# 610265158/Peppa_Pig_Face_Landmark

Measured on NVIDIA H100. Metric: faces/sec Student@256 batch=256, higher is better.
Workload: dtype f32

## Files before the change

### peppa_pig_face_landmark_b200/csrc/conv_tct.cu

```cuda
#include <cuda.h>
#include <cuda_fp16.h>
#include <math.h>
#include <string.h>

#include <algorithm>

#include "../../include/skps_b200.h"
#include "common.h"
#include "conv_tct.h"
#include "tc_ptx.h"

namespace skps {

constexpr int TCT_THREADS = 288;
constexpr int TCT_M = 128, TCT_N = 256;
constexpr int TCT_KC = 32;
constexpr int TCT_W_PLANE = TCT_M * 2 * TCT_KC;
constexpr int TCT_W_SLOT = 2 * TCT_W_PLANE;
constexpr int TCT_W_SLOTS = 3;
constexpr int TCT_MAX_X_SLOTS = 3;
constexpr int TCT_OUT_BYTES = 2 * 16384;
constexpr int TCT_SMEM_LIMIT = 227 * 1024 - 256;

template <int ACT>
__global__ void __launch_bounds__(TCT_THREADS, 1)
conv_tct_kernel(const __grid_constant__ CUtensorMap tmX_hi, const __grid_constant__ CUtensorMap tmX_lo,
                const __grid_constant__ CUtensorMap tmW_hi, const __grid_constant__ CUtensorMap tmW_lo,
                const __grid_constant__ CUtensorMap tmO_hi, const __grid_constant__ CUtensorMap tmO_lo, const TctK p) {
    extern __shared__ uint8_t smem_raw[];
    __shared__ __align__(8) uint64_t full_w[TCT_W_SLOTS], empty_w[TCT_W_SLOTS], full_x[TCT_MAX_X_SLOTS],
        empty_x[TCT_MAX_X_SLOTS];

    const int warp = threadIdx.x >> 5, lane = threadIdx.x & 31;
    const uint32_t base = (smem_u32(smem_raw) + 1023u) & ~1023u;
    const uint32_t x_base = base + (uint32_t)TCT_W_SLOTS * TCT_W_SLOT;
    const uint32_t x_slot = 2u * (uint32_t)p.x_plane;
    const uint32_t out_off = x_base + (uint32_t)p.x_slots * x_slot;
    const int tiles = p.m_tiles;
    const int kh = p.taps / p.kw;
    const int halves = (p.Cin + TCT_KC - 1) / TCT_KC;
    const int groups = p.kw * halves;

    if (warp == 8 && lane == 0) {
        asm volatile("prefetch.tensormap [%0];" ::"l"(&tmX_hi) : "memory");
        asm volatile("prefetch.tensormap [%0];" ::"l"(&tmX_lo) : "memory");
        asm volatile("prefetch.tensormap [%0];" ::"l"(&tmW_hi) : "memory");
        asm volatile("prefetch.tensormap [%0];" ::"l"(&tmW_lo) : "memory");
    }
    if (warp == 1 && lane == 0) {
        for (int s = 0; s < TCT_W_SLOTS; ++s) {
            mbar_init(smem_u32(&full_w[s]), 1);
            mbar_init(smem_u32(&empty_w[s]), 8);
        }
        for (int s = 0; s < p.x_slots; ++s) {
            mbar_init(smem_u32(&full_x[s]), 1);
            mbar_init(smem_u32(&empty_x[s]), 8);
        }
        asm volatile("fence.mbarrier_init.release.cluster;" ::: "memory");
    }
    __syncthreads();

    if (warp == 8) {
        if (lane == 0 && (int)blockIdx.x < tiles) {
            const int total = ((tiles - (int)blockIdx.x + (int)gridDim.x - 1) / (int)gridDim.x) * groups;
            int xs = 0, ws = 0;
            uint32_t xphase = 0, wphase = 0;
            auto load_halo = [&](int n) {
                const int i = n / groups, g = n - i * groups;
                const int kx = g / halves, hc = g - kx * halves;
                const int tile = (int)blockIdx.x + i * (int)gridDim.x;
                const int img_l = tile / p.tiles_per_img, t = tile - img_l * p.tiles_per_img;
                mbar_wait(smem_u32(&empty_x[xs]), xphase ^ 1u);
                const uint32_t fb = smem_u32(&full_x[xs]);
                mbar_expect_tx(fb, x_slot);
                const uint32_t sx = x_base + (uint32_t)xs * x_slot;
                const int cx = kx * p.dil - p.pad, cy = t * p.bh - p.pad;
                tma_load_4d(sx, &tmX_hi, fb, hc * TCT_KC, cx, cy, img_l + p.img0);
                tma_load_4d(sx + (uint32_t)p.x_plane, &tmX_lo, fb, hc * TCT_KC, cx, cy, img_l + p.img0);
                if (++xs == p.x_slots) { xs = 0; xphase ^= 1u; }
            };
            load_halo(0);
            for (int n = 0, g = 0; n < total; ++n) {
                const int kx = g / halves, hc = g - kx * halves;
                for (int ky = 0; ky < kh; ++ky) {
                    mbar_wait(smem_u32(&empty_w[ws]), wphase ^ 1u);
                    const uint32_t fb = smem_u32(&full_w[ws]);
                    mbar_expect_tx(fb, (uint32_t)TCT_W_SLOT);
                    const uint32_t sw = base + (uint32_t)ws * TCT_W_SLOT;
                    const int col = (ky * p.kw + kx) * p.cchunks * 64 + hc * TCT_KC;
                    tma_load_2d(sw, &tmW_hi, fb, col, 0);
                    tma_load_2d(sw + TCT_W_PLANE, &tmW_lo, fb, col, 0);
                    if (++ws == TCT_W_SLOTS) { ws = 0; wphase ^= 1u; }
                    if (ky == 0 && n + 1 < total) load_halo(n + 1);
                }
                if (++g == groups) g = 0;
            }
        }
    } else {
        const int q = warp & 3;
        const int half_id = warp >> 2;
        const bool leader = q == 0 && lane == 0;
        float bias[4];
#pragma unroll
        for (int r = 0; r < 4; ++r) {
            const int c = 64 * (r >> 1) + 16 * q + (lane >> 2) + 8 * (r & 1);
            bias[r] = c < p.Cout ? __ldg(p.bias + c) : 0.f;
        }
        const uint32_t sbuf = out_off + (uint32_t)half_id * 16384u;
        uint32_t row_addr[4];
#pragma unroll
        for (int r = 0; r < 4; ++r) {
            const int cq = 16 * (q & 1) + (lane >> 2) + 8 * (r & 1);
            row_addr[r] = sbuf + (uint32_t)(2 * (r >> 1) + (q >> 1)) * 4096u + (uint32_t)(2 * (lane & 3)) * 64u +
                          (uint32_t)((((cq >> 3) ^ (lane & 3)) & 3) << 4) + (uint32_t)(cq & 7) * 2u;
        }
        const int ks_last = (p.Cin - (halves - 1) * TCT_KC + 15) / 16;
        const uint32_t tap_step = (uint32_t)(p.dil * p.W * 2 * TCT_KC);
        int xs = 0, ws = 0;
        uint32_t xphase = 0, wphase = 0;
        for (int tile = blockIdx.x; tile < tiles; tile += gridDim.x) {
            const int img_l = tile / p.tiles_per_img, t = tile - img_l * p.tiles_per_img;
            float acc[128];
            int prev_w = -1, prev_x = -1;
            for (int g = 0, hc = 0; g < groups; ++g) {
                mbar_wait(smem_u32(&full_x[xs]), xphase);
                const uint32_t xo = x_base + (uint32_t)xs * x_slot + (uint32_t)(half_id * 128 * 2 * TCT_KC);
                const bool two = hc != halves - 1 || ks_last == 2;
                for (int ky = 0; ky < kh; ++ky) {
                    mbar_wait(smem_u32(&full_w[ws]), wphase);
                    const uint32_t sw = base + (uint32_t)ws * TCT_W_SLOT;
                    const uint64_t w_hi = make_smem_desc_sw64(sw), w_lo = make_smem_desc_sw64(sw + TCT_W_PLANE);
                    const uint32_t xk = xo + (uint32_t)ky * tap_step;
                    const uint64_t x_hi = make_smem_desc_sw64(xk), x_lo = make_smem_desc_sw64(xk + (uint32_t)p.x_plane);
                    const uint32_t accumulate = (g | ky) != 0;
                    wg_fence_acc(acc);
                    if (two) {
                        wg_fence(); wg_mma3_128x128<2, 64>(acc, w_hi, w_lo, x_hi, x_lo, accumulate); wg_commit();
                    } else {
                        wg_fence(); wg_mma3_128x128<1, 64>(acc, w_hi, w_lo, x_hi, x_lo, accumulate); wg_commit();
                    }
                    wg_fence_acc(acc);
                    wg_wait<1>();
                    wg_fence_acc(acc);
                    if (lane == 0) {
                        if (prev_w >= 0) mbar_arrive(smem_u32(&empty_w[prev_w]));
                        if (prev_x >= 0) mbar_arrive(smem_u32(&empty_x[prev_x]));
                    }
                    prev_w = ws;
                    prev_x = ky == kh - 1 ? xs : -1;
                    if (++ws == TCT_W_SLOTS) { ws = 0; wphase ^= 1u; }
                }
                if (++xs == p.x_slots) { xs = 0; xphase ^= 1u; }
                if (++hc == halves) hc = 0;
            }
            wg_wait<0>();
            wg_fence_acc(acc);
            if (lane == 0) {
                mbar_arrive(smem_u32(&empty_w[prev_w]));
                mbar_arrive(smem_u32(&empty_x[prev_x]));
            }
#pragma unroll
            for (int ci = 0; ci < 4; ++ci) {
                if (leader) asm volatile("cp.async.bulk.wait_group.read 0;" ::: "memory");
                asm volatile("bar.sync %0, 128;" ::"r"(5 + half_id) : "memory");
#pragma unroll
                for (int m = 0; m < 2; ++m)
#pragma unroll
                    for (int i = 0; i < 4; ++i)
#pragma unroll
                        for (int e = 0; e < 4; ++e) {
                            const float f = act_t<ACT>(fmaf(acc[64 * m + 16 * ci + 4 * i + e], p.out_scale, bias[2 * m + (e >> 1)]));
                            const __half h = __float2half_rn(f);
                            const __half l = __float2half_rn(f - __half2float(h));
                            const uint32_t a = row_addr[2 * m + (e >> 1)] + (uint32_t)(8 * i + (e & 1)) * 64u;
                            asm volatile("st.shared.b16 [%0], %1;" ::"r"(a), "h"(__half_as_ushort(h)) : "memory");
                            asm volatile("st.shared.b16 [%0], %1;" ::"r"(a + 2048u), "h"(__half_as_ushort(l)) : "memory");
                        }
                asm volatile("fence.proxy.async.shared::cta;" ::: "memory");
                asm volatile("bar.sync %0, 128;" ::"r"(5 + half_id) : "memory");
                if (leader) {
                    const int col0 = half_id * 128 + ci * 32;
                    const int x0 = col0 % p.W, y0 = t * p.bh + col0 / p.W;
                    for (int cq = 0; cq < 4 && cq * 32 < p.Cout; ++cq) {
                        const uint32_t sq = sbuf + (uint32_t)cq * 4096u;
                        asm volatile("cp.async.bulk.tensor.4d.global.shared::cta.bulk_group [%0, {%2, %3, %4, %5}], [%1];"
                                     ::"l"(&tmO_hi), "r"(sq), "r"(cq * 32), "r"(x0), "r"(y0), "r"(img_l + p.img0) : "memory");
                        asm volatile("cp.async.bulk.tensor.4d.global.shared::cta.bulk_group [%0, {%2, %3, %4, %5}], [%1];"
                                     ::"l"(&tmO_lo), "r"(sq + 2048u), "r"(cq * 32), "r"(x0), "r"(y0), "r"(img_l + p.img0) : "memory");
                    }
                    asm volatile("cp.async.bulk.commit_group;" ::: "memory");
                }
            }
        }
        if (leader) asm volatile("cp.async.bulk.wait_group 0;" ::: "memory");
    }
}

static int tct_x_plane(const TcSetup& s) { return (TCT_N / s.W + s.dil * (s.kh - 1)) * s.W * 2 * TCT_KC; }
static int tct_x_slots(const TcSetup& s) {
    const int room = TCT_SMEM_LIMIT - 1024 - TCT_W_SLOTS * TCT_W_SLOT - TCT_OUT_BYTES;
    return std::min(TCT_MAX_X_SLOTS, room / (2 * tct_x_plane(s)));
}

bool tct_applicable(const TcSetup& s) {
    const int stride = s.stride > 0 ? s.stride : 1;
    if (stride != 1 || s.kh != s.kw || s.kh < 3 || s.pad != s.dil * (s.kh - 1) / 2) return false;
    if (s.W < 16 || s.W > TCT_N || TCT_N % s.W || s.H % (TCT_N / s.W)) return false;
    if (s.Cin < 64 || (s.Cin % 8) || (s.in_ld % 8) || (s.in_coff % 8)) return false;
    if (s.Cout < 96 || s.Cout > TCT_M || (s.Cout % 8) || s.n_tiles != 1) return false;
    if (s.res || s.hm_val || s.out_fmt != DT_SPLIT16 || s.out_cstride != 1 || (s.out_ld % 8) || (s.out_coff % 8)) return false;
    if (s.act == ACT_SILU) return false;
    return tct_x_slots(s) >= 2;
}

int tct_prepare(TctLayer& L, const TcSetup& s) {
    EncodeTiledFn enc = tensor_map_encoder();
    SKPS_CHECK(enc, "cuTensorMapEncodeTiled entry point not available");
    SKPS_CHECK(tct_applicable(s), "conv_tct: layer not applicable");
    TctK& k = L.k;
    memset(&k, 0, sizeof(k));
    k.W = s.W; k.bh = TCT_N / s.W; k.tiles_per_img = s.H / k.bh;
    k.taps = s.kh * s.kw; k.kw = s.kw; k.dil = s.dil; k.pad = s.pad;
    k.cchunks = (s.Cin + 63) / 64; k.Cin = s.Cin; k.Cout = s.Cout; k.act = s.act; k.out_scale = s.out_scale;
    SKPS_CHECK(s.bias, "conv_tct: bias required");
    k.bias = s.bias;
    k.x_plane = tct_x_plane(s); k.x_slots = tct_x_slots(s);
    L.smem_bytes = 1024 + TCT_W_SLOTS * TCT_W_SLOT + k.x_slots * 2 * k.x_plane + TCT_OUT_BYTES;
    for (int plane = 0; plane < 2; ++plane) {
        cuuint64_t dims[4] = {(cuuint64_t)s.Cin, (cuuint64_t)s.W, (cuuint64_t)s.H, (cuuint64_t)s.max_batch};
        cuuint64_t strides[3] = {(cuuint64_t)s.in_ld * 2, (cuuint64_t)s.W * s.in_ld * 2, (cuuint64_t)s.H * s.W * s.in_ld * 2};
        cuuint32_t box[4] = {TCT_KC, (cuuint32_t)s.W, (cuuint32_t)(k.bh + s.dil * (s.kh - 1)), 1};
        cuuint32_t estr[4] = {1, 1, 1, 1};
        void* base = (void*)((__half*)s.in_base + (plane ? s.in_plane : 0) + s.in_coff);
        CUresult r = enc(plane ? &L.x_lo : &L.x_hi, CU_TENSOR_MAP_DATA_TYPE_FLOAT16, 4, base, dims, strides, box, estr,
                         CU_TENSOR_MAP_INTERLEAVE_NONE, CU_TENSOR_MAP_SWIZZLE_64B,
                         CU_TENSOR_MAP_L2_PROMOTION_L2_128B, CU_TENSOR_MAP_FLOAT_OOB_FILL_NONE);
        SKPS_CHECK(r == CUDA_SUCCESS, "cuTensorMapEncodeTiled(tct X) failed: %d", (int)r);
    }
    const int K_pad = k.taps * k.cchunks * 64;
    for (int plane = 0; plane < 2; ++plane) {
        cuuint64_t dims[2] = {(cuuint64_t)K_pad, (cuuint64_t)s.n_tile};
        cuuint64_t strides[1] = {(cuuint64_t)K_pad * 2};
        cuuint32_t box[2] = {TCT_KC, (cuuint32_t)TCT_M};
        cuuint32_t estr[2] = {1, 1};
        void* base = (void*)(plane ? s.w_lo : s.w_hi);
        CUresult r = enc(plane ? &L.w_lo : &L.w_hi, CU_TENSOR_MAP_DATA_TYPE_FLOAT16, 2, base, dims, strides, box, estr,
                         CU_TENSOR_MAP_INTERLEAVE_NONE, CU_TENSOR_MAP_SWIZZLE_64B,
                         CU_TENSOR_MAP_L2_PROMOTION_L2_256B, CU_TENSOR_MAP_FLOAT_OOB_FILL_NONE);
        SKPS_CHECK(r == CUDA_SUCCESS, "cuTensorMapEncodeTiled(tct W) failed: %d", (int)r);
    }
    for (int plane = 0; plane < 2; ++plane) {
        cuuint64_t dims[4] = {(cuuint64_t)s.Cout, (cuuint64_t)s.W, (cuuint64_t)s.H, (cuuint64_t)s.max_batch};
        cuuint64_t strides[3] = {(cuuint64_t)s.out_ld * 2, (cuuint64_t)s.W * s.out_ld * 2, (cuuint64_t)s.H * s.W * s.out_ld * 2};
        const cuuint32_t obw = (cuuint32_t)(s.W < 32 ? s.W : 32);
        cuuint32_t box[4] = {32, obw, 32 / obw, 1};
        cuuint32_t estr[4] = {1, 1, 1, 1};
        char* base = (char*)s.out + (size_t)s.out_coff * 2 + (plane ? (size_t)s.out_plane * 2 : 0);
        CUresult r = enc(plane ? &L.o_lo : &L.o_hi, CU_TENSOR_MAP_DATA_TYPE_FLOAT16, 4, base, dims, strides, box, estr,
                         CU_TENSOR_MAP_INTERLEAVE_NONE, CU_TENSOR_MAP_SWIZZLE_64B, CU_TENSOR_MAP_L2_PROMOTION_NONE,
                         CU_TENSOR_MAP_FLOAT_OOB_FILL_NONE);
        SKPS_CHECK(r == CUDA_SUCCESS, "cuTensorMapEncodeTiled(tct out) failed: %d", (int)r);
    }
    return 0;
}

template <int ACT>
static int tct_launch_t(const TctLayer& L, const TctK& k, int grid, cudaStream_t stream) {
    static int attr_bytes[MAX_DEVICES] = {};
    if (smem_limit((const void*)conv_tct_kernel<ACT>, attr_bytes, L.smem_bytes)) return 1;
    conv_tct_kernel<ACT><<<grid, TCT_THREADS, L.smem_bytes, stream>>>(L.x_hi, L.x_lo, L.w_hi, L.w_lo, L.o_hi, L.o_lo, k);
    SKPS_CUDA(cudaGetLastError());
    return 0;
}

Grid tct_grid(const TctLayer& L, int batch, int num_sms, TctK* kp) {
    TctK k = L.k;
    k.m_tiles = batch * k.tiles_per_img;
    if (kp) *kp = k;
    return persistent_grid(k.m_tiles, num_sms);
}

int tct_launch(const TctLayer& L, int batch, int num_sms, cudaStream_t stream) {
    TctK k;
    const int grid = tct_grid(L, batch, num_sms, &k).ctas;
    switch (k.act) {
        case ACT_NONE: return tct_launch_t<ACT_NONE>(L, k, grid, stream);
        case ACT_RELU: return tct_launch_t<ACT_RELU>(L, k, grid, stream);
        case ACT_HSWISH: return tct_launch_t<ACT_HSWISH>(L, k, grid, stream);
        case ACT_SIGMOID: return tct_launch_t<ACT_SIGMOID>(L, k, grid, stream);
        case ACT_HSIGMOID: return tct_launch_t<ACT_HSIGMOID>(L, k, grid, stream);
        default: break;
    }
    set_error("conv_tct: activation %d not instantiated", k.act);
    return 1;
}

}
```

Baseline: 20180.

## Multicast conv weight tiles across 2-CTA clusters and shrink output staging

Result: faster. 20510, median of 6 (+1.7%).

```diff
diff --git a/peppa_pig_face_landmark_b200/csrc/conv_tct.cu b/peppa_pig_face_landmark_b200/csrc/conv_tct.cu
--- a/peppa_pig_face_landmark_b200/csrc/conv_tct.cu
+++ b/peppa_pig_face_landmark_b200/csrc/conv_tct.cu
@@ -17,10 +17,42 @@
 constexpr int TCT_KC = 32;
 constexpr int TCT_W_PLANE = TCT_M * 2 * TCT_KC;
 constexpr int TCT_W_SLOT = 2 * TCT_W_PLANE;
-constexpr int TCT_W_SLOTS = 3;
+constexpr int TCT_W_SLOTS = 4;
 constexpr int TCT_MAX_X_SLOTS = 3;
-constexpr int TCT_OUT_BYTES = 2 * 16384;
+constexpr int TCT_OUT_BYTES = 2 * 8192;
 constexpr int TCT_SMEM_LIMIT = 227 * 1024 - 256;
+constexpr int TCT_CLUSTER = 2;
+constexpr int TCT_W_ROWS = TCT_M / TCT_CLUSTER;
+constexpr int TCT_W_BOX = TCT_W_ROWS * 2 * TCT_KC;
+
+__device__ __forceinline__ uint32_t cluster_ctarank() {
+    uint32_t r;
+    asm volatile("mov.u32 %0, %%cluster_ctarank;" : "=r"(r));
+    return r;
+}
+__device__ __forceinline__ uint32_t cluster_nctarank() {
+    uint32_t r;
+    asm volatile("mov.u32 %0, %%cluster_nctarank;" : "=r"(r));
+    return r;
+}
+__device__ __forceinline__ void cluster_sync() {
+    asm volatile("barrier.cluster.arrive.release;\n\tbarrier.cluster.wait.acquire;" ::: "memory");
+}
+__device__ __forceinline__ void mbar_arrive_remote(uint32_t bar, uint32_t rank) {
+    asm volatile(
+        "{\n\t"
+        ".reg .b32 ra;\n\t"
+        "mapa.shared::cluster.u32 ra, %0, %1;\n\t"
+        "mbarrier.arrive.shared::cluster.b64 _, [ra];\n\t"
+        "}\n" ::"r"(bar), "r"(rank) : "memory");
+}
+__device__ __forceinline__ void tma_load_2d_multicast(uint32_t dst, const CUtensorMap* map, uint32_t bar, int c0, int c1,
+                                                      uint16_t mask) {
+    asm volatile(
+        "cp.async.bulk.tensor.2d.shared::cluster.global.mbarrier::complete_tx::bytes.multicast::cluster"
+        " [%0], [%1, {%3, %4}], [%2], %5;"
+        ::"r"(dst), "l"(map), "r"(bar), "r"(c0), "r"(c1), "h"(mask) : "memory");
+}
 
 template <int ACT>
 __global__ void __launch_bounds__(TCT_THREADS, 1)
@@ -40,6 +72,10 @@
     const int kh = p.taps / p.kw;
     const int halves = (p.Cin + TCT_KC - 1) / TCT_KC;
     const int groups = p.kw * halves;
+    const uint32_t nc = cluster_nctarank(), rank = cluster_ctarank();
+    const int grid = (int)gridDim.x;
+    const int mine = (tiles - (int)blockIdx.x + grid - 1) / grid;
+    const int rounds = (tiles - ((int)blockIdx.x - (int)rank) + grid - 1) / grid;
 
     if (warp == 8 && lane == 0) {
         asm volatile("prefetch.tensormap [%0];" ::"l"(&tmX_hi) : "memory");
@@ -50,7 +86,7 @@
     if (warp == 1 && lane == 0) {
         for (int s = 0; s < TCT_W_SLOTS; ++s) {
             mbar_init(smem_u32(&full_w[s]), 1);
-            mbar_init(smem_u32(&empty_w[s]), 8);
+            mbar_init(smem_u32(&empty_w[s]), 8 * nc);
         }
         for (int s = 0; s < p.x_slots; ++s) {
             mbar_init(smem_u32(&full_x[s]), 1);
@@ -58,11 +94,13 @@
         }
         asm volatile("fence.mbarrier_init.release.cluster;" ::: "memory");
     }
-    __syncthreads();
+    if (nc > 1) cluster_sync();
+    else __syncthreads();
 
     if (warp == 8) {
-        if (lane == 0 && (int)blockIdx.x < tiles) {
-            const int total = ((tiles - (int)blockIdx.x + (int)gridDim.x - 1) / (int)gridDim.x) * groups;
+        if (lane == 0 && rounds > 0) {
+            const int total = rounds * groups, x_total = mine * groups;
+            const uint16_t mask = (uint16_t)((1u << nc) - 1u);
             int xs = 0, ws = 0;
             uint32_t xphase = 0, wphase = 0;
             auto load_halo = [&](int n) {
@@ -79,7 +117,7 @@
                 tma_load_4d(sx + (uint32_t)p.x_plane, &tmX_lo, fb, hc * TCT_KC, cx, cy, img_l + p.img0);
                 if (++xs == p.x_slots) { xs = 0; xphase ^= 1u; }
             };
-            load_halo(0);
+            if (x_total > 0) load_halo(0);
             for (int n = 0, g = 0; n < total; ++n) {
                 const int kx = g / halves, hc = g - kx * halves;
                 for (int ky = 0; ky < kh; ++ky) {
@@ -88,10 +126,18 @@
                     mbar_expect_tx(fb, (uint32_t)TCT_W_SLOT);
                     const uint32_t sw = base + (uint32_t)ws * TCT_W_SLOT;
                     const int col = (ky * p.kw + kx) * p.cchunks * 64 + hc * TCT_KC;
-                    tma_load_2d(sw, &tmW_hi, fb, col, 0);
-                    tma_load_2d(sw + TCT_W_PLANE, &tmW_lo, fb, col, 0);
+                    for (int r = (int)rank; r < TCT_CLUSTER; r += (int)nc) {
+                        const uint32_t so = sw + (uint32_t)(r * TCT_W_BOX);
+                        if (nc > 1) {
+                            tma_load_2d_multicast(so, &tmW_hi, fb, col, r * TCT_W_ROWS, mask);
+                            tma_load_2d_multicast(so + TCT_W_PLANE, &tmW_lo, fb, col, r * TCT_W_ROWS, mask);
+                        } else {
+                            tma_load_2d(so, &tmW_hi, fb, col, r * TCT_W_ROWS);
+                            tma_load_2d(so + TCT_W_PLANE, &tmW_lo, fb, col, r * TCT_W_ROWS);
+                        }
+                    }
                     if (++ws == TCT_W_SLOTS) { ws = 0; wphase ^= 1u; }
-                    if (ky == 0 && n + 1 < total) load_halo(n + 1);
+                    if (ky == 0 && n + 1 < x_total) load_halo(n + 1);
                 }
                 if (++g == groups) g = 0;
             }
@@ -106,16 +152,23 @@
             const int c = 64 * (r >> 1) + 16 * q + (lane >> 2) + 8 * (r & 1);
             bias[r] = c < p.Cout ? __ldg(p.bias + c) : 0.f;
         }
-        const uint32_t sbuf = out_off + (uint32_t)half_id * 16384u;
-        uint32_t row_addr[4];
-#pragma unroll
-        for (int r = 0; r < 4; ++r) {
-            const int cq = 16 * (q & 1) + (lane >> 2) + 8 * (r & 1);
-            row_addr[r] = sbuf + (uint32_t)(2 * (r >> 1) + (q >> 1)) * 4096u + (uint32_t)(2 * (lane & 3)) * 64u +
+        const uint32_t sbuf = out_off + (uint32_t)half_id * (uint32_t)(TCT_OUT_BYTES / 2);
+        uint32_t row_addr[2];
+#pragma unroll
+        for (int h = 0; h < 2; ++h) {
+            const int cq = 16 * (q & 1) + (lane >> 2) + 8 * h;
+            row_addr[h] = sbuf + (uint32_t)(q >> 1) * 4096u + (uint32_t)(2 * (lane & 3)) * 64u +
                           (uint32_t)((((cq >> 3) ^ (lane & 3)) & 3) << 4) + (uint32_t)(cq & 7) * 2u;
         }
         const int ks_last = (p.Cin - (halves - 1) * TCT_KC + 15) / 16;
         const uint32_t tap_step = (uint32_t)(p.dil * p.W * 2 * TCT_KC);
+        auto release_w = [&](int s) {
+            if (nc > 1) {
+                for (uint32_t r = 0; r < nc; ++r) mbar_arrive_remote(smem_u32(&empty_w[s]), r);
+            } else {
+                mbar_arrive(smem_u32(&empty_w[s]));
+            }
+        };
         int xs = 0, ws = 0;
         uint32_t xphase = 0, wphase = 0;
         for (int tile = blockIdx.x; tile < tiles; tile += gridDim.x) {
@@ -143,7 +196,7 @@
                     wg_wait<1>();
                     wg_fence_acc(acc);
                     if (lane == 0) {
-                        if (prev_w >= 0) mbar_arrive(smem_u32(&empty_w[prev_w]));
+                        if (prev_w >= 0) release_w(prev_w);
                         if (prev_x >= 0) mbar_arrive(smem_u32(&empty_x[prev_x]));
                     }
                     prev_w = ws;
@@ -156,33 +209,33 @@
             wg_wait<0>();
             wg_fence_acc(acc);
             if (lane == 0) {
-                mbar_arrive(smem_u32(&empty_w[prev_w]));
+                release_w(prev_w);
                 mbar_arrive(smem_u32(&empty_x[prev_x]));
             }
 #pragma unroll
-            for (int ci = 0; ci < 4; ++ci) {
+            for (int ci = 0; ci < 4; ++ci)
+#pragma unroll
+            for (int m = 0; m < 2; ++m) {
                 if (leader) asm volatile("cp.async.bulk.wait_group.read 0;" ::: "memory");
                 asm volatile("bar.sync %0, 128;" ::"r"(5 + half_id) : "memory");
 #pragma unroll
-                for (int m = 0; m < 2; ++m)
-#pragma unroll
-                    for (int i = 0; i < 4; ++i)
-#pragma unroll
-                        for (int e = 0; e < 4; ++e) {
-                            const float f = act_t<ACT>(fmaf(acc[64 * m + 16 * ci + 4 * i + e], p.out_scale, bias[2 * m + (e >> 1)]));
-                            const __half h = __float2half_rn(f);
-                            const __half l = __float2half_rn(f - __half2float(h));
-                            const uint32_t a = row_addr[2 * m + (e >> 1)] + (uint32_t)(8 * i + (e & 1)) * 64u;
-                            asm volatile("st.shared.b16 [%0], %1;" ::"r"(a), "h"(__half_as_ushort(h)) : "memory");
-                            asm volatile("st.shared.b16 [%0], %1;" ::"r"(a + 2048u), "h"(__half_as_ushort(l)) : "memory");
-                        }
+                for (int i = 0; i < 4; ++i)
+#pragma unroll
+                    for (int e = 0; e < 4; ++e) {
+                        const float f = act_t<ACT>(fmaf(acc[64 * m + 16 * ci + 4 * i + e], p.out_scale, bias[2 * m + (e >> 1)]));
+                        const __half h = __float2half_rn(f);
+                        const __half l = __float2half_rn(f - __half2float(h));
+                        const uint32_t a = row_addr[e >> 1] + (uint32_t)(8 * i + (e & 1)) * 64u;
+                        asm volatile("st.shared.b16 [%0], %1;" ::"r"(a), "h"(__half_as_ushort(h)) : "memory");
+                        asm volatile("st.shared.b16 [%0], %1;" ::"r"(a + 2048u), "h"(__half_as_ushort(l)) : "memory");
+                    }
                 asm volatile("fence.proxy.async.shared::cta;" ::: "memory");
                 asm volatile("bar.sync %0, 128;" ::"r"(5 + half_id) : "memory");
                 if (leader) {
                     const int col0 = half_id * 128 + ci * 32;
                     const int x0 = col0 % p.W, y0 = t * p.bh + col0 / p.W;
-                    for (int cq = 0; cq < 4 && cq * 32 < p.Cout; ++cq) {
-                        const uint32_t sq = sbuf + (uint32_t)cq * 4096u;
+                    for (int cq = 2 * m; cq < 2 * m + 2 && cq * 32 < p.Cout; ++cq) {
+                        const uint32_t sq = sbuf + (uint32_t)(cq - 2 * m) * 4096u;
                         asm volatile("cp.async.bulk.tensor.4d.global.shared::cta.bulk_group [%0, {%2, %3, %4, %5}], [%1];"
                                      ::"l"(&tmO_hi), "r"(sq), "r"(cq * 32), "r"(x0), "r"(y0), "r"(img_l + p.img0) : "memory");
                         asm volatile("cp.async.bulk.tensor.4d.global.shared::cta.bulk_group [%0, {%2, %3, %4, %5}], [%1];"
@@ -192,8 +245,14 @@
                 }
             }
         }
+        for (int n = mine * groups * kh; n < rounds * groups * kh; ++n) {
+            mbar_wait(smem_u32(&full_w[ws]), wphase);
+            if (lane == 0) release_w(ws);
+            if (++ws == TCT_W_SLOTS) { ws = 0; wphase ^= 1u; }
+        }
         if (leader) asm volatile("cp.async.bulk.wait_group 0;" ::: "memory");
     }
+    if (nc > 1) cluster_sync();
 }
 
 static int tct_x_plane(const TcSetup& s) { return (TCT_N / s.W + s.dil * (s.kh - 1)) * s.W * 2 * TCT_KC; }
@@ -241,7 +300,7 @@
     for (int plane = 0; plane < 2; ++plane) {
         cuuint64_t dims[2] = {(cuuint64_t)K_pad, (cuuint64_t)s.n_tile};
         cuuint64_t strides[1] = {(cuuint64_t)K_pad * 2};
-        cuuint32_t box[2] = {TCT_KC, (cuuint32_t)TCT_M};
+        cuuint32_t box[2] = {TCT_KC, (cuuint32_t)TCT_W_ROWS};
         cuuint32_t estr[2] = {1, 1};
         void* base = (void*)(plane ? s.w_lo : s.w_hi);
         CUresult r = enc(plane ? &L.w_lo : &L.w_hi, CU_TENSOR_MAP_DATA_TYPE_FLOAT16, 2, base, dims, strides, box, estr,
@@ -264,12 +323,29 @@
     return 0;
 }
 
+static int tct_cluster(int grid) {
+    int c = TCT_CLUSTER;
+    while (grid % c) c >>= 1;
+    return c;
+}
+
 template <int ACT>
 static int tct_launch_t(const TctLayer& L, const TctK& k, int grid, cudaStream_t stream) {
     static int attr_bytes[MAX_DEVICES] = {};
     if (smem_limit((const void*)conv_tct_kernel<ACT>, attr_bytes, L.smem_bytes)) return 1;
-    conv_tct_kernel<ACT><<<grid, TCT_THREADS, L.smem_bytes, stream>>>(L.x_hi, L.x_lo, L.w_hi, L.w_lo, L.o_hi, L.o_lo, k);
-    SKPS_CUDA(cudaGetLastError());
+    cudaLaunchAttribute attr[1];
+    attr[0].id = cudaLaunchAttributeClusterDimension;
+    attr[0].val.clusterDim.x = tct_cluster(grid);
+    attr[0].val.clusterDim.y = 1;
+    attr[0].val.clusterDim.z = 1;
+    cudaLaunchConfig_t cfg = {};
+    cfg.gridDim = dim3(grid);
+    cfg.blockDim = dim3(TCT_THREADS);
+    cfg.dynamicSmemBytes = L.smem_bytes;
+    cfg.stream = stream;
+    cfg.attrs = attr;
+    cfg.numAttrs = 1;
+    SKPS_CUDA(cudaLaunchKernelEx(&cfg, conv_tct_kernel<ACT>, L.x_hi, L.x_lo, L.w_hi, L.w_lo, L.o_hi, L.o_lo, k));
     return 0;
 }
 
```
